# Gallicchio-Lab/openmm_agbnp_plugin

Hardware: AMD Instinct MI355X
Metric: AGBNP1 force-eval-limited ns/day (1 fs step), thrombin 1dwc, independent replicas (higher is better)
Workload: dtype f64

## Files before the change

### openmm_agbnp_plugin_amd/csrc/engine.hip

```cpp
#include <hip/hip_runtime.h>

#include <algorithm>
#include <atomic>
#include <chrono>
#include <cmath>
#include <cstdio>
#include <cstdlib>
#include <cstring>
#include <string>
#include <vector>

#include "../../include/agbnp_hip.h"
#include "adapter_kernels.h"
#include "agbnp_common.h"
#include "i4_tables.h"
#include "pair_kernels.h"
#include "tree_kernels.h"

namespace agbnp {
size_t tree_variant_lds_bytes(int variant);
size_t tree_variant_scratch_bytes(int variant);
int tree_variant_node_cap(int variant);
int tree_variant_atom_cap(int variant);
int tree_variant_wgs_per_cu(int variant);
// ... 774 lines not shown
    }
    if (c->variant > 3 || c->nh <= 0 || c->diagnostics || capturing || (host_set_only && c->five_device)) {
      c->five_active = false;
      c->parity = 0;
      apply_parity(c);
      c->generation++;
    }
  }
  const int tree_grid = std::max(1, std::min(c->slot_cap, c->tree_slots[c->variant]));
  if (c->five_active) {
    hipStreamCaptureStatus cap = hipStreamCaptureStatusNone;
    if (!c->five_device && hipStreamIsCapturing(st, &cap) == hipSuccess && cap != hipStreamCaptureStatusNone) {
      c->five_device = true;
      c->generation++;
    }
    apply_parity(c);
    c->five_evals++;
    c->T.pos = d_pos;
    c->T.out.h2a = c->d_h2a.p;
    const int want_kind = c->P.in.posq ? 1 : 0;
    c->T.posq = c->P.in.posq;
    c->T.posq_corr = c->P.in.correction;
    c->T.posq_double = c->P.in.is_double;
    c->T.hslot = c->P.in.hslot;
    if (c->row_atoms_kind != want_kind) {
      HIP_TRY(c, launch_row_atoms(c->slot_cap, c->d_rows.p, want_kind ? c->d_hslot.p : c->d_h2a.p, c->d_row_atoms.p, st));
      c->row_atoms_kind = want_kind;
    }
    if (!c->masks_valid) {
      HIP_TRY(c, launch_masks(c->P, st, tl));
      c->masks_valid = true;
    }
    if (tl) HIP_TRY(c, tl->mark(kKTreeCavity, st));
    HIP_TRY(c, launch_tree_cavity_five(c->variant, tree_grid, c->T, c->P, st));
  } else {
    HIP_TRY(c, launch_prep(c->P, st, tl));
    if (tl) HIP_TRY(c, tl->mark(kKTreeCavity, st));
    HIP_TRY(c, launch_tree_cavity(c->variant, kGlobalGrid, tree_grid, c->T, st));
  }
  if (c->version == 1) {
    HIP_TRY(c, launch_pair_stages(c->P, d_energy, c->d_components.p, st, tl));
    if (tl) HIP_TRY(c, tl->mark(kKTreePseudo, st));
    TreeOutputs& O = c->T.out;
    static const bool fuse_queued = getenv("AGBNP_HIP_FUSE_QUEUED") && atoi(getenv("AGBNP_HIP_FUSE_QUEUED")) != 0;
    const bool one_round = c->forests_hint > 0 && c->forests_hint <= c->tree_slots[c->variant];
    const bool fused = c->fused_outputs && c->nh > 0 && (c->nh <= 2 * c->tree_slots[c->variant] || one_round || (fuse_queued && c->variant <= 1));
    O.enabled = fused ? 1 : 0;
    O.n = c->n;
    O.a2h = c->d_a2h.p;
    O.h2a = c->d_h2a.p;
    O.force = c->P.omm.force_fixed ? nullptr : d_force;
    O.force_fixed = c->P.omm.force_fixed;
    O.padded = c->P.omm.padded;
    O.ctx_slot = c->P.omm.ctx_slot;
    O.gb_f = c->P.gb_fx;
    O.db_f = c->P.db_fx;
    O.rows_on = c->P.rows_on;
    O.bw = c->P.bw;
    O.grec = c->P.grec;
    O.hrec = c->P.hrec;
    O.nl_flag = c->P.nl_flag;
    O.nl_nitems = c->P.nl_nitems;
    O.row_target = c->P.row_target;
    O.gb_rows = c->P.gb_rows;
    HIP_TRY(c, launch_tree_pseudo(c->variant, kGlobalGrid, tree_grid, c->T, st));
    if (fused) {
      if (tl) HIP_TRY(c, tl->mark(-1, st));
      return AGBNP_HIP_OK;
// ... 698 lines not shown
```

### openmm_agbnp_plugin_amd/csrc/tree_kernels.h

```cpp
#pragma once
#include <hip/hip_runtime.h>

#include <type_traits>

#include "agbnp_common.h"
#include "device_math.h"

namespace agbnp {

enum HeavyRow {
  kHvX = 0, kHvY, kHvZ,
  kHvALarge, kHvVLarge,
  kHvAVdw, kHvVVdw,
  kHvGam,
  kHvInvVol,
  kHvSvLarge,
  kHvGx, kHvGy, kHvGz,
  kHvSvVdw,
  kHvRows
};

struct TreeOutputs {
  int enabled;
  int n;
  int forest_blocks;
  const int *a2h, *h2a;
  double* force;
  unsigned long long* force_fixed;
  int padded;
  const int* ctx_slot;
  const double *gb_f, *db_f;
  int rows_on;
  const double* bw;
  const double4 *grec, *hrec;
  const int* nl_nitems;
  int row_target, gb_rows;
  int* nl_flag;
};

struct PairArgs;

struct TreeArgs {
  TreeOutputs out;
  int nh;
  unsigned hstride;
  double* hv;
  int want_sv_large;
  int det;
  int split_fit;
  const int* rows;
  const int* packing;
  int slot_cap;
  const unsigned long long* nbmask;
  int nhb;
  const double* db_wu;
  double rcut2;
  double* epart;
  SubtreeHeader* hdr;
  int2* sizes;
  unsigned long long* node_pool;
  int* atom_pool;
  unsigned short* pair_pool;
  int* status;
  char* scratch;
  size_t scratch_stride;
  const double* pos;
  const int* row_atoms;
  const void* posq;
  const float4* posq_corr;
  int posq_double;
  const int* hslot;
  int five;
  const int* epoch;
  size_t table_doubles, sizes_stride;

  __device__ __forceinline__ double& hvat(int row, int h) const { return hv[(unsigned)row * hstride + (unsigned)h]; }
  __device__ __forceinline__ const int* forest_start() const { return packing; }
  __device__ __forceinline__ const int* nforests() const { return packing + slot_cap + 1; }
  __device__ __forceinline__ int* cur_nforests() const { return const_cast<int*>(packing) + slot_cap + 2; }
};

// ... 225 lines not shown
  return v;
}

template <int CTRL, int ROW_MASK>
__device__ __forceinline__ double dpp_f64(double v) {
  const unsigned long long u = (unsigned long long)__double_as_longlong(v);
  const unsigned lo = (unsigned)__builtin_amdgcn_update_dpp(0, (int)(unsigned)u, CTRL, ROW_MASK, 0xf, false);
  const unsigned hi = (unsigned)__builtin_amdgcn_update_dpp(0, (int)(unsigned)(u >> 32), CTRL, ROW_MASK, 0xf, false);
  return __longlong_as_double((long long)(((unsigned long long)hi << 32) | lo));
}
__device__ __forceinline__ double wave_sum_f64(double v) {
  v += dpp_f64<0x111, 0xf>(v);
  v += dpp_f64<0x112, 0xf>(v);
  v += dpp_f64<0x114, 0xf>(v);
  v += dpp_f64<0x118, 0xf>(v);
  v += dpp_f64<0x142, 0xa>(v);
  v += dpp_f64<0x143, 0xc>(v);
  const unsigned long long u = (unsigned long long)__double_as_longlong(v);
  const unsigned lo = (unsigned)__builtin_amdgcn_readlane((int)(unsigned)u, 63);
  const unsigned hi = (unsigned)__builtin_amdgcn_readlane((int)(unsigned)(u >> 32), 63);
  return __longlong_as_double((long long)(((unsigned long long)hi << 32) | lo));
}

#ifdef AGBNP_STAMPS
#define AGBNP_BUILD_STAMP(i)                                         \
  do {                                                               \
    if (tid == 0) {                                                  \
      const unsigned long long t_now__ = __builtin_readcyclecounter(); \
      S.stamps[i] += t_now__ - tb_prev__;                            \
      tb_prev__ = t_now__;                                           \
    }                                                                \
  } while (0)
#define AGBNP_BUILD_STAMP_BEGIN() unsigned long long tb_prev__ = __builtin_readcyclecounter()
#else
#define AGBNP_BUILD_STAMP(i)
#define AGBNP_BUILD_STAMP_BEGIN()
#endif

__device__ __forceinline__ unsigned long long kept_bits(const unsigned long long* kmask, int ts, int te) {
  const int len = te - ts;
  if (len <= 0) return 0ull;
  const int c0 = ts >> 6, sh = ts & 63;
  unsigned long long m = kmask[c0] >> sh;
  if (sh + len > 64) m |= kmask[c0 + 1] << (64 - sh);
  return m & ((1ull << len) - 1ull);
}

enum BuildResult { kBuildOk = 0, kBuildNodeOverflow = 1, kBuildAtomOverflow = 2 };

#ifndef AGBNP_WAVE_TAIL
#define AGBNP_WAVE_TAIL 0
#endif
__device__ __forceinline__ void wave_sync() {
  asm volatile("s_waitcnt lgkmcnt(0)" ::: "memory");
  __builtin_amdgcn_wave_barrier();
}
template <int NCAP, int ACAP>
__device__ __forceinline__ bool expand_tail_wave(const TreeStore<NCAP, ACAP>& S, int lane, int L, int level_begin, int& tail_io) {
  constexpr int TCAP = TreeStore<NCAP, ACAP>::TCAP;
  unsigned char* tmap = reinterpret_cast<unsigned char*>(S.cand_vol);
  double* tvol = S.nd[6];
  int tail = tail_io;
  for (; L < kMaxOrder; L++) {
    const int lb = level_begin, le = tail;
    level_begin = le;
    if (lb >= le) break;
    for (int nb = lb; nb < le;) {
// ... 492 lines not shown
            S.ncs[slot] = (unsigned short)(cb + c);
            S.ncc[slot] = 0;
          }
        }
      };
      if (tid < T) create(tid, keep_v, keep_j, keep_ts, keep_te, keep_la);
      for (int t = tid + BS; t < T; t += BS) {
        const int j = tmap[t];
        create(t, tvol[t], j, S.tstart[j], S.tstart[j + 1], -1);
      }
      tree_barrier<NCAP>();
      AGBNP_BUILD_STAMP(13);
      tail += created;
      nb += nin;
    }
  }
#if AGBNP_WAVE_TAIL > 0
  if (tail_from >= 0) {
    if (tid < 64) {
      const bool fits = expand_tail_wave<NCAP, ACAP>(S, tid, L, tail_from, tail);
      if (tid == 0) S.ctl[1] = fits ? tail : -1;
    }
    tree_barrier<NCAP>();
    tail = S.ctl[1];
    if (tail < 0) return kBuildNodeOverflow;
  }
#endif
  tree_barrier<NCAP>();
  *nnodes_out = tail;
  *natoms_out = m + ncand;
  return kBuildOk;
}

template <int NCAP, int ACAP, int BS>
__device__ __forceinline__ void pair_gather(const TreeStore<NCAP, ACAP>& S, int tid, int total, bool with_selfvol, bool det) {
  const int chunk = (total + BS - 1) / BS;
  int k = tid * chunk;
  const int kend = k + chunk < total ? k + chunk : total;
  const int lane = tid & 63;
  int cur = -1, head_atom = -1;
  bool in_first = true;
  double xa = 0.0, ya = 0.0, za = 0.0, ea = 0.0, gx = 0.0, gy = 0.0, gz = 0.0, sv = 0.0;
  double hx = 0.0, hy = 0.0, hz = 0.0, hs = 0.0;
  auto plain_add = [&](int atom, double vx, double vy, double vz, double vs) {
    S.at[6][atom] += vx;
    S.at[7][atom] += vy;
    S.at[8][atom] += vz;
    if (with_selfvol) S.at[9][atom] += vs;
  };
  auto atomic_add = [&](int atom, double vx, double vy, double vz, double vs) {
#ifdef AGBNP_TIMING_GATHER_PLAIN
    return plain_add(atom, vx, vy, vz, vs);
#endif
    lds_add(&S.at[6][atom], vx);
    lds_add(&S.at[7][atom], vy);
    lds_add(&S.at[8][atom], vz);
    if (with_selfvol) lds_add(&S.at[9][atom], vs);
  };
  for (; k < kend; k++) {
    const int pr = S.pairs[k];
    const int a = pr >> 9, n = pr & 511;
    const double cf = S.nd[3][n], cx = S.nd[0][n], cy = S.nd[1][n], cz = S.nd[2][n], wn = S.wrow[n];
    if (a != cur) {
      if (cur >= 0) {
        if (in_first) {
          head_atom = cur, hx = gx, hy = gy, hz = gz, hs = sv;
        } else {
          plain_add(cur, gx, gy, gz, sv);
        }
        in_first = false;
      }
      cur = a;
      xa = S.at[0][a], ya = S.at[1][a], za = S.at[2][a], ea = S.at[3][a];
      gx = gy = gz = sv = 0.0;
    }
    const double am = cf * ea;
    if (det) {
      gx += quantize(am * (xa - cx), kQGrad, true);
      gy += quantize(am * (ya - cy), kQGrad, true);
      gz += quantize(am * (za - cz), kQGrad, true);
    } else {
      gx = fma(am, xa - cx, gx);
      gy = fma(am, ya - cy, gy);
      gz = fma(am, za - cz, gz);
    }
    sv += wn;
  }
  const int key = cur >= 0 ? cur : -2 - lane;
  {
    const int prev_key = __builtin_amdgcn_update_dpp(-1, key, 0x138, 0xf, 0xf, false);
    const bool head_cont = head_atom >= 0 && lane > 0 && prev_key == head_atom;
    if (head_atom >= 0 && !head_cont) {
      if (lane == 0)
        atomic_add(head_atom, hx, hy, hz, hs);
      else
        plain_add(head_atom, hx, hy, hz, hs);
    }
    const double sx = head_cont ? hx : 0.0, sy = head_cont ? hy : 0.0, sz = head_cont ? hz : 0.0, ss = head_cont ? hs : 0.0;
    gx += dpp_f64<0x130, 0xf>(sx);
    gy += dpp_f64<0x130, 0xf>(sy);
    gz += dpp_f64<0x130, 0xf>(sz);
    if (with_selfvol) sv += dpp_f64<0x130, 0xf>(ss);
  }
  auto seg_step = [&](auto ctrl_tag, auto mask_tag) {
    constexpr int CTRL = decltype(ctrl_tag)::value, MASK = decltype(mask_tag)::value;
    const int src_key = __builtin_amdgcn_update_dpp(-1, key, CTRL, MASK, 0xf, false);
    const bool same = src_key == key;
    const double ax = dpp_f64<CTRL, MASK>(gx), ay = dpp_f64<CTRL, MASK>(gy), az = dpp_f64<CTRL, MASK>(gz);
    gx += same ? ax : 0.0;
    gy += same ? ay : 0.0;
    gz += same ? az : 0.0;
    if (with_selfvol) {
      const double as = dpp_f64<CTRL, MASK>(sv);
      sv += same ? as : 0.0;
    }
  };
  seg_step(std::integral_constant<int, 0x111>{}, std::integral_constant<int, 0xf>{});
  seg_step(std::integral_constant<int, 0x112>{}, std::integral_constant<int, 0xf>{});
  seg_step(std::integral_constant<int, 0x114>{}, std::integral_constant<int, 0xf>{});
  seg_step(std::integral_constant<int, 0x118>{}, std::integral_constant<int, 0xf>{});
  seg_step(std::integral_constant<int, 0x142>{}, std::integral_constant<int, 0xa>{});
  seg_step(std::integral_constant<int, 0x143>{}, std::integral_constant<int, 0xc>{});
  {
    const int next_key = __builtin_amdgcn_update_dpp(-1, key, 0x130, 0xf, 0xf, false);
    const bool seg_end = cur >= 0 && (lane == 63 || next_key != key);
    const int key_first = __builtin_amdgcn_readfirstlane(key), key_last = __builtin_amdgcn_readlane(key, 63);
    if (seg_end) {
      if (key == key_first || key == key_last)
        atomic_add(cur, gx, gy, gz, sv);
      else
        plain_add(cur, gx, gy, gz, sv);
    }
  }
}

__device__ __forceinline__ double pi_power(int k) {
  const double p2 = kPi * kPi, p4 = p2 * p2;
  double r = (k & 1) ? kPi : 1.0;
  r = (k & 2) ? r * p2 : r;
  r = (k & 4) ? r * p4 : r;
  return r;
}

struct NoHook {
  __device__ __forceinline__ void operator()() const {}
};
template <int NCAP, int ACAP, int BS, bool WITH_ENERGY, bool FRESH_BUILD = false, class AfterPairs = NoHook>
__device__ bool volume_pass(const TreeStore<NCAP, ACAP>& S, int tid, int m, int nnodes, int natoms, bool with_selfvol,
                            double* e_sum, int* npairs, bool det, const uint4* pair_word = nullptr, AfterPairs after_pairs = AfterPairs()) {
  static_assert(ACAP <= 256, "atom path stores one byte per level");
  static_assert(BS % 64 == 0 && BS >= 64, "whole waves");
  constexpr bool kPairs = TreeStore<NCAP, ACAP>::kPairGather;
  constexpr int PCAP = TreeStore<NCAP, ACAP>::PCAP;
  unsigned long long* path = reinterpret_cast<unsigned long long*>(S.nd[6]);
  AGBNP_BUILD_STAMP_BEGIN();
  if (FRESH_BUILD && kPairs) {
    for (int la = tid; la < ACAP; la += BS) S.pcnt[la] = 0;
    tree_barrier<NCAP>();
  }
  constexpr unsigned long long kPartners = 0x00ffffffffffffffull;
  double e_part = 0.0;
  for (int nbase = m; nbase < nnodes; nbase += BS) {
    const int n = nbase + tid;
    int level = 0, rootq = -1;
    double g = 0.0, gam = 0.0, w = 0.0;
    do {
      if (n >= nnodes) break;
    if (FRESH_BUILD) {
      {
        const int par = S.npar[n];
        if (par < m) {
          const int pp = S.rt[kRtPart + par];
          if (level2_owner(n - S.rt[kRtBase + par], pp >> 8) != (pp & 0xff)) {
            path[n] = (unsigned long long)par << 56;
            S.nd[3][n] = 0.0;
            S.wrow[n] = 0.0;
            break;
          }
        }
      }
// ... 11 lines not shown
      gam += S.at[5][rootq];
      path[n] = pw | ((unsigned long long)rootq << 56);
      g = S.nd[4][n];
    } else {
      const unsigned long long pwr = path[n];
      if ((pwr & kPartners) == 0ull) {
        S.nd[3][n] = 0.0;
        S.wrow[n] = 0.0;
        break;
      }
      rootq = (int)(pwr >> 56);
      double A = S.at[3][rootq], cx = S.at[0][rootq], cy = S.at[1][rootq], cz = S.at[2][rootq];
      double pv = S.at[4][rootq], pa = A, E = 0.0;
      gam = S.at[5][rootq];
      level = 1;
      for (unsigned long long pw = pwr & kPartners; pw; pw >>= 8) {
        const int la = (int)(pw & 0xffull);
        const double xk = S.at[0][la], yk = S.at[1][la], zk = S.at[2][la], ak = S.at[3][la];
        const double dx = xk - cx, dy = yk - cy, dz = zk - cz;
        const double inv = fast_rcp(A + ak);
        const double wk = ak * inv;
        E = fma(A * wk, fma(dz, dz, fma(dy, dy, dx * dx)), E);
        cx = fma(dx, wk, cx);
        cy = fma(dy, wk, cy);
        cz = fma(dz, wk, cz);
        A += ak;
        pa *= ak;
        pv *= S.at[4][la];
        gam += S.at[5][la];
        level++;
      }
      const double q = pa * fast_rcp(A * pi_power(level - 1));
      g = pv * pow_three_halves(q) * exp_nonpositive(-E);
      S.nd[0][n] = cx;
      S.nd[1][n] = cy;
      S.nd[2][n] = cz;
    }
    const double cp = ((level & 1) ? 1.0 : -1.0) / (double)level;
    double sp;
    const double sw = dev_switch(g, sp);
    w = quantize(cp * sw * g, kQVol, det);
    S.nd[3][n] = -2.0 * cp * gam * (sp * g + sw) * g;
    S.wrow[n] = w;
    e_part += quantize(gam * (cp * sw * g), kQEnergy, det);
    } while (false);
    if (with_selfvol || FRESH_BUILD) {
      for (unsigned long long todo = __ballot(rootq >= 0); todo;) {
        const int q = __builtin_amdgcn_readlane(rootq, __builtin_ctzll(todo));
        const unsigned long long mine = __ballot(rootq == q);
        if (with_selfvol) {
          const double sq = wave_sum_f64(rootq == q ? w : 0.0);
          if ((tid & 63) == 0) lds_add(&S.at[9][q], sq);
        }
        if (FRESH_BUILD && (tid & 63) == 0) atomicAdd(&S.rt[kRtNodes + q], (int)__popcll(mine));
        todo &= ~mine;
      }
    }
  }
  if (WITH_ENERGY) {
    e_part = wave_sum_f64(e_part);
    if ((tid & 63) == 0) S.misc[tid >> 6] = e_part;
  }
  tree_barrier<NCAP>();
  if (WITH_ENERGY) {
    double es = 0.0;
    for (int w = 0; w < BS / 64; w++) es += S.misc[w];
    *e_sum = es;
  }
  AGBNP_BUILD_STAMP(7);
  if (kPairs) {
    if (FRESH_BUILD) {
      static_assert(!kPairs || ACAP <= 128, "two atoms per lane");
      if (tid < 64) {
        const int a0 = 2 * tid, a1 = 2 * tid + 1;
        const int c0 = a0 < ACAP ? S.pcnt[a0] : 0, c1 = a1 < ACAP ? S.pcnt[a1] : 0;
        const int incl = wave_inclusive_scan(c0 + c1);
        if (a0 < ACAP) S.pcnt[a0] = incl - c0 - c1;
        if (a1 < ACAP) S.pcnt[a1] = incl - c1;
        if (tid == 63) S.ctl[4] = incl;
      }
      tree_barrier<NCAP>();
      const int total = S.ctl[4];
      *npairs = total;
      if (total > PCAP) return false;
      for (int n = m + tid; n < nnodes; n += BS)
        for (unsigned long long pw = path[n] & kPartners; pw; pw >>= 8) {
          const int la = (int)(pw & 0xffull);
          S.pairs[atomicAdd(&S.pcnt[la], 1)] = (unsigned short)((la << 9) | n);
        }
      tree_barrier<NCAP>();
    }
    if (pair_word) {
#pragma unroll
      for (int k = 0; k < (PCAP / 8 + BS - 1) / BS; k++)
        if (tid + k * BS < PCAP / 8) reinterpret_cast<uint4*>(S.pairs)[tid + k * BS] = pair_word[k];
      tree_barrier<NCAP>();
      after_pairs();
    }
    pair_gather<NCAP, ACAP, BS>(S, tid, *npairs, with_selfvol, det);
    tree_barrier<NCAP>();
    AGBNP_BUILD_STAMP(14);
    return true;
  }
  {
    const int A = natoms <= 16 ? 16 : (natoms <= 32 ? 32 : 64);
    const int nslices = BS / A;
    const int slice = tid / A, al = tid - slice * A;
    for (int abase = 0; abase < natoms; abase += A) {
      const int a = abase + al;
      const bool live = a >= m && a < natoms;
      const int aa_idx = live ? a : 0;
      const double xa = S.at[0][aa_idx], ya = S.at[1][aa_idx], za = S.at[2][aa_idx], ea = S.at[3][aa_idx];
      const unsigned long long pat = 0x0101010101010101ull * (unsigned long long)aa_idx;
      double gx = 0.0, gy = 0.0, gz = 0.0, sv = 0.0;
      for (int n = m + slice; n < nnodes; n += nslices) {
        const unsigned long long x = path[n] ^ pat;
        const double cf = S.nd[3][n], cx = S.nd[0][n], cy = S.nd[1][n], cz = S.nd[2][n], wn = S.wrow[n];
        const bool member = live && (((x - 0x0101010101010101ull) & ~x & 0x8080808080808080ull) != 0ull);
        const double am = member ? cf * ea : 0.0;
        gx += quantize(am * (xa - cx), kQGrad, det);
        gy += quantize(am * (ya - cy), kQGrad, det);
        gz += quantize(am * (za - cz), kQGrad, det);
        sv += member ? wn : 0.0;
      }
      for (int off = A; off < 64; off <<= 1) {
        gx += __shfl_xor(gx, off, 64);
        gy += __shfl_xor(gy, off, 64);
        gz += __shfl_xor(gz, off, 64);
        sv += __shfl_xor(sv, off, 64);
      }
      constexpr bool kSingleRound = ACAP <= 64;
      static_assert(kSingleRound || NCAP >= 4 * BS, "exchange area");
      double* ex0 = kSingleRound ? S.nd[0] : S.nd[4];
      double* ex1 = kSingleRound ? S.nd[1] : S.nd[4] + BS;
      double* ex2 = kSingleRound ? S.nd[2] : S.nd[4] + 2 * BS;
      double* ex3 = kSingleRound ? S.nd[3] : S.nd[4] + 3 * BS;
      tree_barrier<NCAP>();
      const int wave = tid >> 6, lane = tid & 63;
      if (lane < A) {
        ex0[wave * 64 + lane] = gx;
        ex1[wave * 64 + lane] = gy;
        ex2[wave * 64 + lane] = gz;
        ex3[wave * 64 + lane] = sv;
      }
      tree_barrier<NCAP>();
      if (tid < A && live) {
        double tx = 0.0, ty = 0.0, tz = 0.0, tv = 0.0;
        for (int w = 0; w < BS / 64; w++) {
          tx += ex0[w * 64 + tid];
          ty += ex1[w * 64 + tid];
          tz += ex2[w * 64 + tid];
          tv += ex3[w * 64 + tid];
        }
        S.at[6][a] += tx;
        S.at[7][a] += ty;
        S.at[8][a] += tz;
        if (with_selfvol) S.at[9][a] += tv;
      }
    }
  }
  tree_barrier<NCAP>();
  AGBNP_BUILD_STAMP(14);
  return true;
}

template <int NCAP, int ACAP, int BS>
__device__ void root_gradients_from_invariance(const TreeStore<NCAP, ACAP>& S, int tid, int m) {
  const int wave = tid >> 6, lane = tid & 63;
  for (int q = wave; q < m; q += BS / 64) {
    const int b = S.rt[kRtBase + q], e = b + S.rt[kRtCount + q];
    double sx = 0.0, sy = 0.0, sz = 0.0;
    for (int la = b + lane; la < e; la += 64) {
      sx += S.at[6][la];
      sy += S.at[7][la];
      sz += S.at[8][la];
    }
    sx = wave_sum_f64(sx);
    sy = wave_sum_f64(sy);
    sz = wave_sum_f64(sz);
    if (lane == 0) {
      S.at[6][q] = -sx;
      S.at[7][q] = -sy;
      S.at[8][q] = -sz;
    }
  }
  tree_barrier<NCAP>();
}

}
```

### openmm_agbnp_plugin_amd/csrc/tree_kernels.hip

```cpp
#include "tree_kernels.h"

#include "pair_kernels.h"
#include "prep_role.h"
#include "row_kernels.h"

namespace agbnp {

#ifdef AGBNP_STAMPS
__device__ unsigned long long g_stamps[16];
__device__ unsigned long long g_stamps_max[16];
__device__ unsigned long long g_stamps_slowest[24];
constexpr int kWgLogSlots = 8192;
__device__ unsigned long long g_wg_log[kWgLogSlots][24];
#define STAMP_BEGIN()                                   \
  if (tid < 16) S.stamps[tid] = 0;                      \
  __syncthreads();                                      \
  const unsigned long long t_wall0__ = wall_clock64();  \
  const unsigned long long t_cyc0__ = __builtin_readcyclecounter(); \
  unsigned long long t_prev__ = __builtin_readcyclecounter()
#define STAMP(i)                                                   \
  do {                                                             \
    lds_barrier();                                                 \
    if (tid == 0) {                                                \
      const unsigned long long t_now__ = __builtin_readcyclecounter(); \
// ... 34 lines not shown
#define CSTAMP_BEGIN()
#define CSTAMP(i)
#define CSTAMP_FLUSH()
#define PSTAMP_BEGIN() STAMP_BEGIN()
#define PSTAMP(i) STAMP(i)
#define PSTAMP_FLUSH() STAMP_FLUSH()
#else
#define CSTAMP_BEGIN() STAMP_BEGIN()
#define CSTAMP(i) STAMP(i)
#define CSTAMP_FLUSH() STAMP_FLUSH()
#define PSTAMP_BEGIN()
#define PSTAMP(i)
#define PSTAMP_FLUSH()
#endif

__device__ __forceinline__ int next_forest(int tid, int* lds_word, int ticket, int grid) {
  if (tid == 0) *lds_word = grid + ticket;
  lds_barrier();
  const int slot = *lds_word;
  lds_barrier();
  return slot;
}

constexpr int tree_waves_per_simd(int ncap, int bs) {
  if (bs == 192) return ncap <= 512 ? 4 : 2;
  return bs >= 256 ? (ncap <= 432 ? 5 : (ncap <= 512 ? 4 : 2)) : (ncap <= 192 ? 3 : 2);
}

#ifdef AGBNP_STAMPS
constexpr int kPendCap = 4;
#else
constexpr int kPendCap = 16;
#endif
template <int NCAP, int ACAP, int BS, bool GLOBAL, bool SV1, bool FIVE, bool POSQ = false>
__device__ __forceinline__ void cavity_forests(const TreeArgs& A, const int tree_blocks) {
  extern __shared__ __align__(16) char smem[];
  TreeStore<NCAP, ACAP> S;
  S.carve(GLOBAL ? (A.scratch + (size_t)blockIdx.x * A.scratch_stride) : smem);
  __shared__ int s_next;
  __shared__ int s_pend[kPendCap + 2];
  int& s_npend = s_pend[kPendCap];
  int& s_out = s_pend[kPendCap + 1];
  const int tid = threadIdx.x;
  int first_item = -1, first_atom = 0;
  if ((tid & 63) < kMaxRoots) first_item = A.rows[(size_t)kRowStride * blockIdx.x + (tid & 63)];
  if (FIVE && (tid & 63) < kMaxRoots) first_atom = A.row_atoms[(size_t)kMaxItems * blockIdx.x + (tid & 63)];
  const int nforests = min(A.nforests()[0], A.slot_cap);
  if (blockIdx.x == 0 && tid == 0) A.cur_nforests()[0] = nforests;
  if ((int)blockIdx.x >= nforests && tid == 0) {
    A.hdr[blockIdx.x].nnodes = 0;
    A.hdr[blockIdx.x].natoms = 0;
  }

  const bool queued = nforests > tree_blocks;
  const int lane = tid & 63;
  for (int slot = blockIdx.x; slot < nforests;) {
    constexpr int kNotAsked = 0x3fffffff;
    int ticket = kNotAsked;
    int my_item = first_item, my_atom = first_atom;
    if (slot != (int)blockIdx.x) {
      int lane_q = lane;
      asm volatile("" : "+v"(lane_q));
      my_item = -1;
      if (lane_q < kMaxRoots) my_item = A.rows[(size_t)kRowStride * slot + lane_q];
      if (FIVE && lane_q < kMaxRoots) my_atom = A.row_atoms[(size_t)kMaxItems * slot + lane_q];
    }
    if (tid == 0) s_npend = 0, s_out = slot;
// ... 100 lines not shown
        SubtreeHeader h;
        h.nnodes = nnodes;
        h.natoms = natoms;
        h.nroots = m;
        h.npairs = npairs;
        for (int q = 0; q < kMaxRoots; q++) h.partners[q] = q < m ? S.rt[kRtCount + q] : 0;
        A.hdr[out] = h;
      }
      if (tid < m) {
        const bool first = (S.rt[kRtPart + tid] & 0xff) == 0;
        int* sz = reinterpret_cast<int*>(&A.sizes[S.rt[kRtHeavy + tid]]);
        atomicAdd(&sz[0], S.rt[kRtNodes + tid] + (first ? 1 : 0));
        if (first) sz[1] = 1 + S.rt[kRtCount + tid];
      }
    }
    CSTAMP(2);
    if (ACAP <= BS) {
      if (tid < natoms) {
        S.at[3][tid] = a_vdw_mine;
        S.at[4][tid] = v_vdw_mine;
        S.at[5][tid] = -S.at[5][tid];
      }
    } else {
      for (int la = tid; la < natoms; la += BS) {
        const int hj = S.at_gidx[la];
        S.at[3][la] = A.hvat(kHvAVdw, hj);
        S.at[4][la] = A.hvat(kHvVVdw, hj);
        S.at[5][la] = -S.at[5][la];
      }
    }
    tree_barrier<NCAP>();
    CSTAMP(3);

    volume_pass<NCAP, ACAP, BS, true>(S, tid, m, nnodes, natoms, true, &e_sum, &npairs, det);
    CSTAMP(4);
    root_gradients_from_invariance<NCAP, ACAP, BS>(S, tid, m);
    CSTAMP(5);

    for (int la = tid; la < natoms; la += BS) {
      const int hj = S.at_gidx[la];
      glb_add(&A.hvat(kHvGx, hj), S.at[6][la]);
      glb_add(&A.hvat(kHvGy, hj), S.at[7][la]);
      glb_add(&A.hvat(kHvGz, hj), S.at[8][la]);
      glb_add(&A.hvat(kHvSvVdw, hj),
              (la < m && (S.rt[kRtPart + la] & 0xff) == 0) ? S.at[9][la] + quantize(S.at[4][la], kQVol, det) : S.at[9][la]);
    }
    if (tid == 0) {
      double e2 = e_sum;
      for (int q = 0; q < m; q++) e2 += (S.rt[kRtPart + q] & 0xff) == 0 ? quantize(S.at[5][q] * S.at[4][q], kQEnergy, det) : 0.0;
      if (out == slot)
        A.epart[2 * slot + 1] = e2;
      else
        A.epart[2 * slot + 1] += e2;
    }
    tree_barrier<NCAP>();
    CSTAMP(6);
    CSTAMP_FLUSH();
    const int npend = s_npend;
    if (npend == 0) break;
    {
      if (tid == 0) s_next = atomicAdd(&A.status[kStatSpareForests], 1);
      lds_barrier();
      const int spare = max(nforests, tree_blocks) + s_next;
      lds_barrier();
      if (spare >= A.slot_cap) {
        if (tid == 0) {
          atomicAdd(&A.status[kStatPackOverflow], 1);
          atomicAdd(&A.status[kStatForestOverflow], 1);
        }
        break;
      }
      const int take = min(npend, kMaxRoots);
      my_item = lane < take ? s_pend[npend - take + lane] : -1;
      if (FIVE) my_atom = my_item >= 0 ? (POSQ ? A.hslot : A.out.h2a)[work_item_root(my_item)] : 0;
      lds_barrier();
      if (tid == 0) s_npend = npend - take, s_out = spare;
    }
    }
    if (!queued) break;
    slot = __builtin_amdgcn_readfirstlane(next_forest(tid, &s_next, ticket, tree_blocks));
  }
}

template <int NCAP, int ACAP, int BS, bool GLOBAL, bool SV1>
__global__ __launch_bounds__(BS, tree_waves_per_simd(NCAP, BS)) void k_tree_cavity(TreeArgs A) {
  cavity_forests<NCAP, ACAP, BS, GLOBAL, SV1, false>(A, (int)gridDim.x);
}

static_assert(kPrepHvGx == kHvGx && kPrepHvGx + 3 == kHvSvVdw && kPrepHvSvLarge == kHvSvLarge, "prep_role.h addresses the table's rows by number");
template <int NCAP, int ACAP, int BS, bool DEVPAR = false, bool POSQ = false>
__global__ __launch_bounds__(BS, tree_waves_per_simd(NCAP, BS)) void k_tree_cavity_five(TreeArgs A, PairArgs P, int tree_blocks) {
  if ((int)blockIdx.x >= tree_blocks) {
    const int b = (int)blockIdx.x - tree_blocks;
    if (DEVPAR) rebase_for_parity(P, 0);
    return prep_atoms(P, b * BS + (int)threadIdx.x, b == 0, true);
  }
  if (DEVPAR) rebase_tree_for_parity(A, 0);
  cavity_forests<NCAP, ACAP, BS, false, false, true, POSQ>(A, tree_blocks);
}

__device__ __forceinline__ bool evaluation_void(const int* __restrict__ status) {
  return (status[kStatNodeOverflow] | status[kStatAtomOverflow] | status[kStatPackOverflow] | status[kStatRowOverflow] | status[kStatOrderStale]) != 0;
}
__device__ __forceinline__ void add_force(const TreeOutputs& O, int atom, double fx, double fy, double fz) {
  if (O.force_fixed) {
    auto to_fixed = [](double f) { return (unsigned long long)(long long)rint(f * 4294967296.0); };
    const int s = O.ctx_slot[atom];
    atomicAdd(&O.force_fixed[s], to_fixed(fx));
    atomicAdd(&O.force_fixed[s + O.padded], to_fixed(fy));
    atomicAdd(&O.force_fixed[s + 2 * O.padded], to_fixed(fz));
  } else {
    glb_add(&O.force[3 * atom], fx);
    glb_add(&O.force[3 * atom + 1], fy);
    glb_add(&O.force[3 * atom + 2], fz);
  }
}
__device__ __forceinline__ void outputs_role(const TreeArgs& A, int blk, int bs) {
  const TreeOutputs& O = A.out;
  const int i = blk * bs + (int)threadIdx.x;
  if (O.rows_on && i == 0) {
    rows_close_evaluation(O.nl_flag, O.nl_nitems, O.row_target, O.gb_rows != 0);
  }
  if (i >= O.n) return;
  const int h = O.a2h[i];
  double fx = 0.0, fy = 0.0, fz = 0.0;
  if (h >= 0) fx = -A.hvat(kHvGx, h), fy = -A.hvat(kHvGy, h), fz = -A.hvat(kHvGz, h);
  const size_t n = (size_t)O.n;
  if (O.rows_on) {
    const double bwi = O.bw[i];
    const double4 g = O.grec[i];
    double sh = 0.0;
// ... 30 lines not shown
  constexpr bool kPipelined = PIPE && !GLOBAL && NCAP <= 8 * BS && ACAP <= BS && TreeStore<NCAP, ACAP>::kPairGather;
  if constexpr (kPipelined) {
    constexpr int KP = (NCAP + BS - 1) / BS;
    constexpr int kPairWordsP = TreeStore<NCAP, ACAP>::PCAP / 8;
    constexpr int kPairRegsP = (kPairWordsP + BS - 1) / BS;
    unsigned long long pw[KP];
    uint4 pair_word[kPairRegsP];
    int hj_pre = 0;
    int h_nnodes = 0, h_natoms = 0, h_m = 0, h_npairs = 0, h_partners[kMaxRoots];
    auto request_topology = [&](int slot_) {
      const SubtreeHeader* H = &A.hdr[slot_];
      const size_t pool_off = (size_t)slot_ * NCAP, atom_off = (size_t)slot_ * ACAP;
#pragma unroll
      for (int k = 0; k < kPairRegsP; k++) {
        pair_word[k] = make_uint4(0, 0, 0, 0);
        if (tid + k * BS < kPairWordsP)
          pair_word[k] = reinterpret_cast<const uint4*>(A.pair_pool + (size_t)slot_ * TreeStore<NCAP, ACAP>::PCAP)[tid + k * BS];
      }
#pragma unroll
      for (int k = 0; k < KP; k++) pw[k] = tid + k * BS < NCAP ? A.node_pool[pool_off + tid + k * BS] : 0ull;
      hj_pre = tid < ACAP ? A.atom_pool[atom_off + tid] : 0;
      h_nnodes = H->nnodes, h_natoms = H->natoms, h_m = H->nroots, h_npairs = H->npairs;
#pragma unroll
      for (int q = 0; q < kMaxRoots; q++) h_partners[q] = H->partners[q];
    };
    double px = 0.0, py = 0.0, pz = 0.0, pa = 0.0, pv = 0.0, pnu = 0.0;
    int pidx = 0;
    auto request_parameters = [&]() {
      if (tid < h_natoms) {
        const int hj = hj_pre;
        px = A.hvat(kHvX, hj), py = A.hvat(kHvY, hj), pz = A.hvat(kHvZ, hj);
        pa = A.hvat(kHvAVdw, hj), pv = A.hvat(kHvVVdw, hj);
        pnu = A.db_wu[hj] * A.hvat(kHvInvVol, hj);
        pidx = write_forces ? A.out.h2a[hj] : 0;
      }
    };
    const bool queued = nforests > grid;
    const bool det = A.det != 0;
    const bool is_void = write_forces && evaluation_void(A.status);
    request_topology(block);
    bool have_parameters = false;
    for (int slot = block;;) {
      PSTAMP_BEGIN();
      const int nnodes = h_nnodes, natoms = h_natoms, m = h_m;
      int npairs = h_npairs;
      if (nnodes <= m) {
        if (!queued) break;
        int ticket = 0;
        if (tid == 0) ticket = atomicAdd(&A.status[kStatPseudoQueue], 1);
        const int slot_ = __builtin_amdgcn_readfirstlane(next_forest(tid, &s_next, ticket, grid));
        if (slot_ >= nforests) break;
        request_topology(slot_);
        have_parameters = false;
        slot = slot_;
        continue;
      }
      if (tid == 0) {
        int run = m;
        for (int q = 0; q < m; q++) {
          S.rt[kRtCount + q] = h_partners[q];
          S.rt[kRtBase + q] = run;
          run += h_partners[q];
        }
      }
      {
        unsigned long long* path = reinterpret_cast<unsigned long long*>(S.nd[6]);
// ... 92 lines not shown
    int npairs = H->npairs;
    const bool queued = nforests > grid;
    if (nnodes <= m) {
      if (queued && tid == 0) ticket = atomicAdd(&A.status[kStatPseudoQueue], 1);
      break;
    }
    if (tid == 0) {
      int run = m;
      for (int q = 0; q < m; q++) {
        const int c = H->partners[q];
        S.rt[kRtCount + q] = c;
        S.rt[kRtBase + q] = run;
        run += c;
      }
    }
    {
      unsigned long long* path = reinterpret_cast<unsigned long long*>(S.nd[6]);
      if (!kPrefetch) {
        for (int n = m + tid; n < nnodes; n += BS) path[n] = A.node_pool[pool_off + n];
      } else {
#pragma unroll
        for (int k = 0; k < (NCAP + BS - 1) / BS; k++)
          if (tid + k * BS >= m && tid + k * BS < nnodes) path[tid + k * BS] = pw[k];
      }
    }
    for (int la = tid; la < natoms; la += BS) {
      const int hj = kPrefetch ? hj_pre : A.atom_pool[atom_off + la];
      S.at_gidx[la] = hj;
      S.at[0][la] = A.hvat(kHvX, hj);
      S.at[1][la] = A.hvat(kHvY, hj);
      S.at[2][la] = A.hvat(kHvZ, hj);
      S.at[3][la] = A.hvat(kHvAVdw, hj);
      S.at[4][la] = A.hvat(kHvVVdw, hj);
      S.at[5][la] = A.db_wu[hj] * A.hvat(kHvInvVol, hj);
      S.at[6][la] = 0.0;
      S.at[7][la] = 0.0;
      S.at[8][la] = 0.0;
      S.at[9][la] = write_forces ? __hiloint2double(0, A.out.h2a[hj]) : 0.0;
    }
    tree_barrier<NCAP>();
    PSTAMP(0);
    if (queued && tid == 0) ticket = atomicAdd(&A.status[kStatPseudoQueue], 1);
    double e_sum = 0.0;
    volume_pass<NCAP, ACAP, BS, false>(S, tid, m, nnodes, natoms, false, &e_sum, &npairs, A.det != 0, kPairs ? pair_word : nullptr);
    PSTAMP(1);
    root_gradients_from_invariance<NCAP, ACAP, BS>(S, tid, m);
    if (write_forces) {
      if (!evaluation_void(A.status)) {
        if (A.out.force_fixed) {
          for (int la = tid; la < natoms; la += BS) add_force(A.out, __double2loint(S.at[9][la]), -S.at[6][la], -S.at[7][la], -S.at[8][la]);
        } else {
          for (int k = tid; k < 3 * natoms; k += BS) {
            const int la = k / 3, c = k - 3 * la;
            const double* row = c == 0 ? S.at[6] : (c == 1 ? S.at[7] : S.at[8]);
            glb_add(&A.out.force[3 * (size_t)__double2loint(S.at[9][la]) + c], -row[la]);
          }
        }
      }
    } else {
      for (int la = tid; la < natoms; la += BS) {
        const int hj = S.at_gidx[la];
        glb_add(&A.hvat(kHvGx, hj), S.at[6][la]);
        glb_add(&A.hvat(kHvGy, hj), S.at[7][la]);
        glb_add(&A.hvat(kHvGz, hj), S.at[8][la]);
      }
    }
    tree_barrier<NCAP>();
// ... 94 lines not shown
  const bool sv1 = A.want_sv_large != 0;
#define AGBNP_CAVITY(...) (sv1 ? launch_tree(k_tree_cavity<__VA_ARGS__, true>, grid, lds, A, st) : launch_tree(k_tree_cavity<__VA_ARGS__, false>, grid, lds, A, st))
  int grid = slots;
  size_t lds = 0;
  switch (variant) {
    case 0: lds = TreeStore<AGBNP_SMALL_STORE>::kBytes; return AGBNP_CAVITY(AGBNP_SMALL_STORE, kBS, false);
    case 1: lds = TreeStore<512, 64>::kBytes; return AGBNP_CAVITY(512, 64, kBS, false);
    case 2: lds = TreeStore<1024, 128>::kBytes; return AGBNP_CAVITY(1024, 128, kBS, false);
    case 3: lds = TreeStore<2048, 256>::kBytes; return AGBNP_CAVITY(2048, 256, kBS, false);
    default: grid = global_grid < A.nh ? global_grid : A.nh; return AGBNP_CAVITY(kGlobalNodeCap, kGlobalAtomCap, kBS, true);
  }
#undef AGBNP_CAVITY
}

template <class K>
static hipError_t launch_five(K kernel, dim3 grid, size_t lds, const TreeArgs& A, const PairArgs& P, int slots, hipStream_t st) {
  if (lds > 48 * 1024) {
    hipError_t e = hipFuncSetAttribute(reinterpret_cast<const void*>(kernel), hipFuncAttributeMaxDynamicSharedMemorySize, (int)lds);
    if (e != hipSuccess) return e;
  }
  hipLaunchKernelGGL(kernel, grid, dim3(kBS), lds, st, A, P, slots);
  return hipGetLastError();
}

hipError_t launch_tree_cavity_five(int variant, int slots, const TreeArgs& A, const PairArgs& P, hipStream_t st) {
  if (A.nh <= 0 || variant > 3) return hipErrorInvalidValue;
  const int work = std::max(std::max(P.n, P.nslots), (int)kStatEvalWords);
  const int prep_blocks = (work + kBS - 1) / kBS;
  const bool dev = A.five == 2, posq = A.posq != nullptr;
  const dim3 grid(slots + prep_blocks);
#define AGBNP_FIVE(NC, AC)                                                                                              \
  do {                                                                                                                 \
    const size_t lds = TreeStore<NC, AC>::kBytes;                                                                      \
    if (dev && posq) return launch_five(k_tree_cavity_five<NC, AC, kBS, true, true>, grid, lds, A, P, slots, st);      \
    if (dev) return launch_five(k_tree_cavity_five<NC, AC, kBS, true, false>, grid, lds, A, P, slots, st);             \
    if (posq) return launch_five(k_tree_cavity_five<NC, AC, kBS, false, true>, grid, lds, A, P, slots, st);            \
    return launch_five(k_tree_cavity_five<NC, AC, kBS, false, false>, grid, lds, A, P, slots, st);                     \
  } while (0)
  switch (variant) {
    case 0: AGBNP_FIVE(kSmallNodes, kSmallAtoms);
    case 1: AGBNP_FIVE(512, 64);
    case 2: AGBNP_FIVE(1024, 128);
    default: AGBNP_FIVE(2048, 256);
  }
#undef AGBNP_FIVE
}

hipError_t launch_tree_pseudo(int variant, int global_grid, int slots, const TreeArgs& A0, hipStream_t st) {
  if (A0.nh <= 0) return hipSuccess;
  TreeArgs A = A0;
  A.out.forest_blocks = variant <= 3 ? slots : (global_grid < A.nh ? global_grid : A.nh);
  const int grid = A.out.forest_blocks + (A.out.enabled ? (A.out.n + kBS - 1) / kBS : 0);
  switch (variant) {
    case 0:
      if (A.five == 2 && A.out.enabled) return launch_tree(k_tree_pseudo<AGBNP_SMALL_STORE, kBS, false, false, true>, grid, TreeStore<AGBNP_SMALL_STORE>::kReplayBytes, A, st);
      if (A.five == 2) return launch_tree(k_tree_pseudo<AGBNP_SMALL_STORE, kBS, false, true, true>, grid, TreeStore<AGBNP_SMALL_STORE>::kReplayBytes, A, st);
      if (A.out.enabled) return launch_tree(k_tree_pseudo<AGBNP_SMALL_STORE, kBS, false, false>, grid, TreeStore<AGBNP_SMALL_STORE>::kReplayBytes, A, st);
      return launch_tree(k_tree_pseudo<AGBNP_SMALL_STORE, kBS, false>, grid, TreeStore<AGBNP_SMALL_STORE>::kReplayBytes, A, st);
    case 1:
      if (A.five == 2 && A.out.enabled) return launch_tree(k_tree_pseudo<512, 64, kBS, false, false, true>, grid, TreeStore<512, 64>::kReplayBytes, A, st);
      if (A.five == 2) return launch_tree(k_tree_pseudo<512, 64, kBS, false, true, true>, grid, TreeStore<512, 64>::kReplayBytes, A, st);
      if (A.out.enabled) return launch_tree(k_tree_pseudo<512, 64, kBS, false, false>, grid, TreeStore<512, 64>::kReplayBytes, A, st);
      return launch_tree(k_tree_pseudo<512, 64, kBS, false>, grid, TreeStore<512, 64>::kReplayBytes, A, st);
    case 2:
      if (A.five == 2) return launch_tree(k_tree_pseudo<1024, 128, kBS, false, true, true>, grid, TreeStore<1024, 128>::kReplayBytes, A, st);
      return launch_tree(k_tree_pseudo<1024, 128, kBS, false>, grid, TreeStore<1024, 128>::kReplayBytes, A, st);
// ... 9 lines not shown
```

Before: 879.9.

## Defer cavity-pass gradients into pseudo pass by folding gamma into atom weights

When the fused five-stage path runs with version 1, the cavity volume pass skips computing and gathering per-node gradient terms, templated off through a new GRAD flag. The later pseudo-volume pass subtracts each atom's gamma from its weight so that the cavity gradient contribution is recovered algebraically in a single gradient sweep. This removes duplicated gradient accumulation, LDS stores and DPP reductions in the cavity kernel. It relies on the linearity of the gradient in the per-atom weights and doubles the number of kernel instantiations.

Measured after the change: 891.7, median of 6. 1.01x the previous value.

```diff
diff --git a/openmm_agbnp_plugin_amd/csrc/engine.hip b/openmm_agbnp_plugin_amd/csrc/engine.hip
--- a/openmm_agbnp_plugin_amd/csrc/engine.hip
+++ b/openmm_agbnp_plugin_amd/csrc/engine.hip
@@ -830,8 +830,10 @@
       c->masks_valid = true;
     }
     if (tl) HIP_TRY(c, tl->mark(kKTreeCavity, st));
+    c->T.defer_grad = c->version == 1 ? 1 : 0;
     HIP_TRY(c, launch_tree_cavity_five(c->variant, tree_grid, c->T, c->P, st));
   } else {
+    c->T.defer_grad = 0;
     HIP_TRY(c, launch_prep(c->P, st, tl));
     if (tl) HIP_TRY(c, tl->mark(kKTreeCavity, st));
     HIP_TRY(c, launch_tree_cavity(c->variant, kGlobalGrid, tree_grid, c->T, st));
diff --git a/openmm_agbnp_plugin_amd/csrc/tree_kernels.h b/openmm_agbnp_plugin_amd/csrc/tree_kernels.h
--- a/openmm_agbnp_plugin_amd/csrc/tree_kernels.h
+++ b/openmm_agbnp_plugin_amd/csrc/tree_kernels.h
@@ -47,6 +47,7 @@
   double* hv;
   int want_sv_large;
   int det;
+  int defer_grad;
   int split_fit;
   const int* rows;
   const int* packing;
@@ -338,7 +339,12 @@
     }                                                                \
   } while (0)
 #define AGBNP_BUILD_STAMP_BEGIN() unsigned long long tb_prev__ = __builtin_readcyclecounter()
+#define AGBNP_BUILD_STAMP_SKIP() \
+  do {                           \
+    if (tid == 0) tb_prev__ = __builtin_readcyclecounter(); \
+  } while (0)
 #else
+#define AGBNP_BUILD_STAMP_SKIP()
 #define AGBNP_BUILD_STAMP(i)
 #define AGBNP_BUILD_STAMP_BEGIN()
 #endif
@@ -897,7 +903,7 @@
   return kBuildOk;
 }
 
-template <int NCAP, int ACAP, int BS>
+template <int NCAP, int ACAP, int BS, bool GRAD = true>
 __device__ __forceinline__ void pair_gather(const TreeStore<NCAP, ACAP>& S, int tid, int total, bool with_selfvol, bool det) {
   const int chunk = (total + BS - 1) / BS;
   int k = tid * chunk;
@@ -908,24 +914,29 @@
   double xa = 0.0, ya = 0.0, za = 0.0, ea = 0.0, gx = 0.0, gy = 0.0, gz = 0.0, sv = 0.0;
   double hx = 0.0, hy = 0.0, hz = 0.0, hs = 0.0;
   auto plain_add = [&](int atom, double vx, double vy, double vz, double vs) {
-    S.at[6][atom] += vx;
-    S.at[7][atom] += vy;
-    S.at[8][atom] += vz;
+    if (GRAD) {
+      S.at[6][atom] += vx;
+      S.at[7][atom] += vy;
+      S.at[8][atom] += vz;
+    }
     if (with_selfvol) S.at[9][atom] += vs;
   };
   auto atomic_add = [&](int atom, double vx, double vy, double vz, double vs) {
 #ifdef AGBNP_TIMING_GATHER_PLAIN
     return plain_add(atom, vx, vy, vz, vs);
 #endif
-    lds_add(&S.at[6][atom], vx);
-    lds_add(&S.at[7][atom], vy);
-    lds_add(&S.at[8][atom], vz);
+    if (GRAD) {
+      lds_add(&S.at[6][atom], vx);
+      lds_add(&S.at[7][atom], vy);
+      lds_add(&S.at[8][atom], vz);
+    }
     if (with_selfvol) lds_add(&S.at[9][atom], vs);
   };
   for (; k < kend; k++) {
     const int pr = S.pairs[k];
     const int a = pr >> 9, n = pr & 511;
-    const double cf = S.nd[3][n], cx = S.nd[0][n], cy = S.nd[1][n], cz = S.nd[2][n], wn = S.wrow[n];
+    const double cf = GRAD ? S.nd[3][n] : 0.0, cx = GRAD ? S.nd[0][n] : 0.0, cy = GRAD ? S.nd[1][n] : 0.0, cz = GRAD ? S.nd[2][n] : 0.0,
+                 wn = S.wrow[n];
     if (a != cur) {
       if (cur >= 0) {
         if (in_first) {
@@ -936,11 +947,12 @@
         in_first = false;
       }
       cur = a;
-      xa = S.at[0][a], ya = S.at[1][a], za = S.at[2][a], ea = S.at[3][a];
+      if (GRAD) xa = S.at[0][a], ya = S.at[1][a], za = S.at[2][a], ea = S.at[3][a];
       gx = gy = gz = sv = 0.0;
     }
     const double am = cf * ea;
-    if (det) {
+    if (!GRAD) {
+    } else if (det) {
       gx += quantize(am * (xa - cx), kQGrad, true);
       gy += quantize(am * (ya - cy), kQGrad, true);
       gz += quantize(am * (za - cz), kQGrad, true);
@@ -962,19 +974,23 @@
         plain_add(head_atom, hx, hy, hz, hs);
     }
     const double sx = head_cont ? hx : 0.0, sy = head_cont ? hy : 0.0, sz = head_cont ? hz : 0.0, ss = head_cont ? hs : 0.0;
-    gx += dpp_f64<0x130, 0xf>(sx);
-    gy += dpp_f64<0x130, 0xf>(sy);
-    gz += dpp_f64<0x130, 0xf>(sz);
+    if (GRAD) {
+      gx += dpp_f64<0x130, 0xf>(sx);
+      gy += dpp_f64<0x130, 0xf>(sy);
+      gz += dpp_f64<0x130, 0xf>(sz);
+    }
     if (with_selfvol) sv += dpp_f64<0x130, 0xf>(ss);
   }
   auto seg_step = [&](auto ctrl_tag, auto mask_tag) {
     constexpr int CTRL = decltype(ctrl_tag)::value, MASK = decltype(mask_tag)::value;
     const int src_key = __builtin_amdgcn_update_dpp(-1, key, CTRL, MASK, 0xf, false);
     const bool same = src_key == key;
-    const double ax = dpp_f64<CTRL, MASK>(gx), ay = dpp_f64<CTRL, MASK>(gy), az = dpp_f64<CTRL, MASK>(gz);
-    gx += same ? ax : 0.0;
-    gy += same ? ay : 0.0;
-    gz += same ? az : 0.0;
+    if (GRAD) {
+      const double ax = dpp_f64<CTRL, MASK>(gx), ay = dpp_f64<CTRL, MASK>(gy), az = dpp_f64<CTRL, MASK>(gz);
+      gx += same ? ax : 0.0;
+      gy += same ? ay : 0.0;
+      gz += same ? az : 0.0;
+    }
     if (with_selfvol) {
       const double as = dpp_f64<CTRL, MASK>(sv);
       sv += same ? as : 0.0;
@@ -1010,7 +1026,7 @@
 struct NoHook {
   __device__ __forceinline__ void operator()() const {}
 };
-template <int NCAP, int ACAP, int BS, bool WITH_ENERGY, bool FRESH_BUILD = false, class AfterPairs = NoHook>
+template <int NCAP, int ACAP, int BS, bool WITH_ENERGY, bool FRESH_BUILD = false, bool GRAD = true, class AfterPairs = NoHook>
 __device__ bool volume_pass(const TreeStore<NCAP, ACAP>& S, int tid, int m, int nnodes, int natoms, bool with_selfvol,
                             double* e_sum, int* npairs, bool det, const uint4* pair_word = nullptr, AfterPairs after_pairs = AfterPairs()) {
   static_assert(ACAP <= 256, "atom path stores one byte per level");
@@ -1088,15 +1104,17 @@
       }
       const double q = pa * fast_rcp(A * pi_power(level - 1));
       g = pv * pow_three_halves(q) * exp_nonpositive(-E);
-      S.nd[0][n] = cx;
-      S.nd[1][n] = cy;
-      S.nd[2][n] = cz;
+      if (GRAD) {
+        S.nd[0][n] = cx;
+        S.nd[1][n] = cy;
+        S.nd[2][n] = cz;
+      }
     }
     const double cp = ((level & 1) ? 1.0 : -1.0) / (double)level;
     double sp;
     const double sw = dev_switch(g, sp);
     w = quantize(cp * sw * g, kQVol, det);
-    S.nd[3][n] = -2.0 * cp * gam * (sp * g + sw) * g;
+    if (GRAD) S.nd[3][n] = -2.0 * cp * gam * (sp * g + sw) * g;
     S.wrow[n] = w;
     e_part += quantize(gam * (cp * sw * g), kQEnergy, det);
     } while (false);
@@ -1123,7 +1141,7 @@
     for (int w = 0; w < BS / 64; w++) es += S.misc[w];
     *e_sum = es;
   }
-  AGBNP_BUILD_STAMP(7);
+  if (!FRESH_BUILD) AGBNP_BUILD_STAMP(7);
   if (kPairs) {
     if (FRESH_BUILD) {
       static_assert(!kPairs || ACAP <= 128, "two atoms per lane");
@@ -1153,11 +1171,13 @@
       tree_barrier<NCAP>();
       after_pairs();
     }
-    pair_gather<NCAP, ACAP, BS>(S, tid, *npairs, with_selfvol, det);
+    if (FRESH_BUILD) AGBNP_BUILD_STAMP_SKIP();
+    pair_gather<NCAP, ACAP, BS, GRAD>(S, tid, *npairs, with_selfvol, det);
     tree_barrier<NCAP>();
-    AGBNP_BUILD_STAMP(14);
+    AGBNP_BUILD_STAMP(FRESH_BUILD ? 15 : 14);
     return true;
   }
+  if (FRESH_BUILD) AGBNP_BUILD_STAMP_SKIP();
   {
     const int A = natoms <= 16 ? 16 : (natoms <= 32 ? 32 : 64);
     const int nslices = BS / A;
@@ -1173,7 +1193,7 @@
         const unsigned long long x = path[n] ^ pat;
         const double cf = S.nd[3][n], cx = S.nd[0][n], cy = S.nd[1][n], cz = S.nd[2][n], wn = S.wrow[n];
         const bool member = live && (((x - 0x0101010101010101ull) & ~x & 0x8080808080808080ull) != 0ull);
-        const double am = member ? cf * ea : 0.0;
+        const double am = (GRAD && member) ? cf * ea : 0.0;
         gx += quantize(am * (xa - cx), kQGrad, det);
         gy += quantize(am * (ya - cy), kQGrad, det);
         gz += quantize(am * (za - cz), kQGrad, det);
@@ -1208,15 +1228,17 @@
           tz += ex2[w * 64 + tid];
           tv += ex3[w * 64 + tid];
         }
-        S.at[6][a] += tx;
-        S.at[7][a] += ty;
-        S.at[8][a] += tz;
+        if (GRAD) {
+          S.at[6][a] += tx;
+          S.at[7][a] += ty;
+          S.at[8][a] += tz;
+        }
         if (with_selfvol) S.at[9][a] += tv;
       }
     }
   }
   tree_barrier<NCAP>();
-  AGBNP_BUILD_STAMP(14);
+  AGBNP_BUILD_STAMP(FRESH_BUILD ? 15 : 14);
   return true;
 }
 
diff --git a/openmm_agbnp_plugin_amd/csrc/tree_kernels.hip b/openmm_agbnp_plugin_amd/csrc/tree_kernels.hip
--- a/openmm_agbnp_plugin_amd/csrc/tree_kernels.hip
+++ b/openmm_agbnp_plugin_amd/csrc/tree_kernels.hip
@@ -90,7 +90,7 @@
 #else
 constexpr int kPendCap = 16;
 #endif
-template <int NCAP, int ACAP, int BS, bool GLOBAL, bool SV1, bool FIVE, bool POSQ = false>
+template <int NCAP, int ACAP, int BS, bool GLOBAL, bool SV1, bool FIVE, bool POSQ = false, bool DEFER = false>
 __device__ __forceinline__ void cavity_forests(const TreeArgs& A, const int tree_blocks) {
   extern __shared__ __align__(16) char smem[];
   TreeStore<NCAP, ACAP> S;
@@ -257,7 +257,7 @@
     tree_barrier<NCAP>();
     CSTAMP(3);
 
-    volume_pass<NCAP, ACAP, BS, true>(S, tid, m, nnodes, natoms, true, &e_sum, &npairs, det);
+    volume_pass<NCAP, ACAP, BS, true, false, !DEFER>(S, tid, m, nnodes, natoms, true, &e_sum, &npairs, det);
     CSTAMP(4);
     root_gradients_from_invariance<NCAP, ACAP, BS>(S, tid, m);
     CSTAMP(5);
@@ -313,7 +313,7 @@
 }
 
 static_assert(kPrepHvGx == kHvGx && kPrepHvGx + 3 == kHvSvVdw && kPrepHvSvLarge == kHvSvLarge, "prep_role.h addresses the table's rows by number");
-template <int NCAP, int ACAP, int BS, bool DEVPAR = false, bool POSQ = false>
+template <int NCAP, int ACAP, int BS, bool DEVPAR = false, bool POSQ = false, bool DEFER = false>
 __global__ __launch_bounds__(BS, tree_waves_per_simd(NCAP, BS)) void k_tree_cavity_five(TreeArgs A, PairArgs P, int tree_blocks) {
   if ((int)blockIdx.x >= tree_blocks) {
     const int b = (int)blockIdx.x - tree_blocks;
@@ -321,7 +321,7 @@
     return prep_atoms(P, b * BS + (int)threadIdx.x, b == 0, true);
   }
   if (DEVPAR) rebase_tree_for_parity(A, 0);
-  cavity_forests<NCAP, ACAP, BS, false, false, true, POSQ>(A, tree_blocks);
+  cavity_forests<NCAP, ACAP, BS, false, false, true, POSQ, DEFER>(A, tree_blocks);
 }
 
 __device__ __forceinline__ bool evaluation_void(const int* __restrict__ status) {
@@ -418,6 +418,7 @@
         px = A.hvat(kHvX, hj), py = A.hvat(kHvY, hj), pz = A.hvat(kHvZ, hj);
         pa = A.hvat(kHvAVdw, hj), pv = A.hvat(kHvVVdw, hj);
         pnu = A.db_wu[hj] * A.hvat(kHvInvVol, hj);
+        if (A.defer_grad) pnu -= A.hvat(kHvGam, hj);
         pidx = write_forces ? A.out.h2a[hj] : 0;
       }
     };
@@ -576,7 +577,7 @@
       S.at[2][la] = A.hvat(kHvZ, hj);
       S.at[3][la] = A.hvat(kHvAVdw, hj);
       S.at[4][la] = A.hvat(kHvVVdw, hj);
-      S.at[5][la] = A.db_wu[hj] * A.hvat(kHvInvVol, hj);
+      S.at[5][la] = A.db_wu[hj] * A.hvat(kHvInvVol, hj) - (A.defer_grad ? A.hvat(kHvGam, hj) : 0.0);
       S.at[6][la] = 0.0;
       S.at[7][la] = 0.0;
       S.at[8][la] = 0.0;
@@ -737,6 +738,12 @@
 #define AGBNP_FIVE(NC, AC)                                                                                              \
   do {                                                                                                                 \
     const size_t lds = TreeStore<NC, AC>::kBytes;                                                                      \
+    if (A.defer_grad) {                                                                                                \
+      if (dev && posq) return launch_five(k_tree_cavity_five<NC, AC, kBS, true, true, true>, grid, lds, A, P, slots, st); \
+      if (dev) return launch_five(k_tree_cavity_five<NC, AC, kBS, true, false, true>, grid, lds, A, P, slots, st);     \
+      if (posq) return launch_five(k_tree_cavity_five<NC, AC, kBS, false, true, true>, grid, lds, A, P, slots, st);    \
+      return launch_five(k_tree_cavity_five<NC, AC, kBS, false, false, true>, grid, lds, A, P, slots, st);             \
+    }                                                                                                                  \
     if (dev && posq) return launch_five(k_tree_cavity_five<NC, AC, kBS, true, true>, grid, lds, A, P, slots, st);      \
     if (dev) return launch_five(k_tree_cavity_five<NC, AC, kBS, true, false>, grid, lds, A, P, slots, st);             \
     if (posq) return launch_five(k_tree_cavity_five<NC, AC, kBS, false, true>, grid, lds, A, P, slots, st);            \
```
